# arclab-hku/ESVIO

Hardware: AMD Instinct MI355X
Metric: Mevents/s through time-surface+detect+track @640x480 (higher is better)
Workload: dtype f64 timestamps / u8 images / f32 LK sums in the reference build's order

## Files before the change

### esvio_amd/csrc/fe_api.cpp

```cpp
#include "fe_internal.h"

namespace {
typedef int (*nccl_allgather_fn)(const void*, void*, size_t, int , void* ,
                                 hipStream_t);
struct NcclId {
  char internal[128];
};
typedef int (*nccl_get_id_fn)(NcclId*);
typedef int (*nccl_init_rank_fn)(void** , int, NcclId, int);
typedef int (*nccl_destroy_fn)(void*);
void* rccl_lib() {
  static void* lib = []() -> void* {
    const char* names[] = {"librccl.so.1", "librccl.so"};
    for (const char* n : names)
      if (void* l = dlopen(n, RTLD_NOW | RTLD_NOLOAD | RTLD_GLOBAL)) return l;
    for (const char* n : names)
      if (void* l = dlopen(n, RTLD_NOW | RTLD_GLOBAL)) return l;
    return dlopen("/opt/rocm/lib/librccl.so.1", RTLD_NOW | RTLD_GLOBAL);
  }();
  return lib;
}
template <class F>
F rccl_sym(const char* name) {
  void* l = rccl_lib();
// ... 116 lines not shown
  if (hipSetDevice(dev) != hipSuccess) return ESVIO_FE_ENODEVICE;

  esvio_fe_ctx* c = new esvio_fe_ctx();
  c->cfg = *cfg;
  c->dev = dev;
  c->W = cfg->width;
  c->H = cfg->height;
  c->P = (uint32_t)c->W * c->H;
  c->invalid_key = 2 * c->P;
  c->key_bits = 1;
  while ((1ull << c->key_bits) <= (unsigned long long)c->invalid_key) c->key_bits++;
  c->hw = host::disc_halfwidths(cfg->min_dist);
  c->trace = getenv("ESVIO_FE_TRACE") != nullptr;
  if (const char* v = getenv("ESVIO_FE_SLOW_CALL_MS")) c->slow_call_ms = atof(v);
  c->mask_event.reset(c->W, c->H);

  auto bail = [&](int rc) {
    esvio_fe_destroy(c);
    return rc;
  };
  {
    int n_cu = 0;
    if (hipDeviceGetAttribute(&n_cu, hipDeviceAttributeMultiprocessorCount, dev) != hipSuccess || n_cu <= 0) {
      (void)hipGetLastError();
      n_cu = 64;
    }
    const int lk_blocks = (std::max(cfg->max_cnt, 1) + kLkPointsPerBlock - 1) / kLkPointsPerBlock;
    c->n_cu = n_cu;
    c->waits_fit_spec = lk_blocks + 2 <= n_cu;
    c->waits_fit_chain = 2 * lk_blocks + 2 <= n_cu;
// ... 3425 lines not shown
    for (int i = 0; i <= kMaxDiscR; i++) sa.hw[i] = i < (int)hw.size() ? (int8_t)hw[i] : -1;
  }
  sa.disc_c = (flags & ESVIO_FE_SELECT_TABLE) ? -1 : disc_threshold(sa.hw, sa.radius);
  if (mask) {
    host::BitMask bm;
    bm.reset(c->W, c->H);
    bm.from_bytes(mask);
    std::memcpy(pin.mask, bm.bits.data(), bm.bits.size() * 4);
    HIPCHK(c, hipMemcpyAsync(c->d_mask_bits, pin.mask, bm.bits.size() * 4, hipMemcpyHostToDevice, s));
    sa.init_bits = c->d_mask_bits;
  }
  if (n_stamp) {
    std::memcpy(pin.news, stamp_xy, (size_t)n_stamp * 8);
    sa.stamp_pts = (const float2*)zpin.news;
    sa.n_stamp = n_stamp;
  }
  pin.counts[0] = pin.counts[1] = pin.counts[2] = -1;
  sa.host_counts = zpin.counts;
  if (variant == 1) sa.one_wave = 1;
  if (variant == 2) sa.gbitmap = c->d_sel_bitmap;
  const KernelId id = launch_select_args(c, sa);
  HIPCHK(c, hipMemcpyAsync(out_xy, c->d_ptsD, (size_t)M * 8, hipMemcpyDeviceToHost, s));
  HIPCHK(c, hipMemcpyAsync(out_idx, c->d_sel_idx, (size_t)M * 4, hipMemcpyDeviceToHost, s));
  HIPCHK(c, hipStreamSynchronize(s));
  for (int i = 0; i < 3; i++) counts[i] = pin.counts[i];
  if (kernel_id) *kernel_id = (int32_t)id;
  if (c->prof_on) resolve_profile(c);
  return 0;
}

int esvio_fe_track_image_space(esvio_fe_handle c, double cur_time, const uint8_t* img_left, const uint8_t* img_right, int space,
                               int pub_this_frame, esvio_fe_tracks* out) {
  if (!c || !img_left) return ESVIO_FE_EINVAL;
  if (space != ESVIO_FE_HOST && space != ESVIO_FE_DEVICE) return fail(c, ESVIO_FE_EINVAL, "track_image_space: bad memory space");
  HIPCHK(c, hipSetDevice(c->dev));
  if (!c->announced.empty() || !c->inflight.empty())
    return fail(c, ESVIO_FE_EINVAL, "event batches are announced on this handle");
  if (int rc = track_image_impl(c, cur_time, img_left, img_right, pub_this_frame != 0, space)) return rc;
  return fill_tracks(c, out);
}

int esvio_fe_track_image(esvio_fe_handle c, double cur_time, const uint8_t* img_left,
// ... 787 lines not shown
```

### esvio_amd/csrc/fe_ctx.h

```cpp
#pragma once
#include <hip/hip_runtime.h>

#include <algorithm>
#include <atomic>
#include <chrono>
#include <cmath>
#include <cstdarg>
#include <cstdio>
#include <cstdlib>
#include <cstring>
#include <dlfcn.h>
#include <map>
#include <string>
#include <utility>
#include <deque>
#include <vector>

#include "../../include/esvio_fe.h"
#include "../../include/esvio_fe_test.h"
#include "fe_aedat.h"
#include "fe_bag.h"
#include "fe_host.h"
#include "fe_kernels.h"
#include "fe_layout.h"
// ... 273 lines not shown
  DevBuf<int32_t> d_sel_idx;
  DevBuf<uint8_t> d_fast_img;
  PinBuf<uint8_t> h_img;
  DevBuf<uint8_t> d_img;
  unsigned img_stage_next = 0;
  PinBuf<uint8_t> h_pin;

  int n_id = 0;
  double cur_time = 0, prev_time = 0;
  std::vector<P2f> prev_pts, cur_pts, cur_right_pts, n_pts;
  std::vector<P2f> cur_un_pts, cur_un_right_pts, pts_velocity, right_pts_velocity;
  std::vector<int> ids, ids_right, track_cnt, track_cnt_right;
  std::vector<int> src_idx;
  IdMap cur_un_pts_map, prev_un_pts_map, cur_un_right_pts_map, prev_un_right_pts_map;
  host::BitMask mask_event;

  DevBuf<uint8_t> d_eq_tmp;
  bool select_ok = true;
  bool select_one_wave = false;
  DevBuf<uint32_t> d_sel_bitmap;
  bool trace = false;
  double trace_phase_ms[2][ESVIO_FE_LATENCY_PHASES] = {};
  double tail_ms[2][4] = {};
  uint64_t phase_count[2] = {0, 0};
  uint64_t phase_frames = 0, tr_cand = 0, tr_new = 0, tr_detect = 0, tr_surv = 0;
  uint64_t tr_fm_class[3] = {};
  double tr_fm_ms = 0;
  double tr_fm_max_ms = 0, tr_lift_ms = 0;
  uint64_t tr_chain_launch = 0, tr_chain_used = 0, tr_chain_cancel = 0, tr_spec_used = 0;
  Event ev_dbg_sel_start;
// ... 331 lines not shown
```

### esvio_amd/csrc/fe_host.cpp

```cpp
#include "fe_host.h"

#include <algorithm>
#include <cfloat>
#include <climits>
#include <cmath>
#include <cstdio>
#include <cstdlib>
#include <cstring>

#include <atomic>
#include <chrono>
#include <condition_variable>
#include <sys/resource.h>
#include <memory>
#include <mutex>
#include <thread>

#if defined(__linux__)
#include <pthread.h>
#include <sched.h>
#endif

#if defined(__HIP_DEVICE_COMPILE__) || defined(ESVIO_NO_SIMD_CLONES)
#define ESVIO_SIMD_CLONES
// ... 107 lines not shown

void BitMask::stamp_disc(int cx, int cy, int r, const std::vector<int>& hw) {
  for (int oy = -r; oy <= r; oy++) {
    const int y = cy + oy;
    if (y < 0 || y >= H) continue;
    const int h = hw[oy < 0 ? -oy : oy];
    if (h < 0) continue;
    const int x0 = std::max(cx - h, 0), x1 = std::min(cx + h, W - 1);
    if (x1 < x0) continue;
    for (int w = x0 >> 5; w <= (x1 >> 5); w++) {
      const int lo = std::max(x0 - (w << 5), 0), hi = std::min(x1 - (w << 5), 31);
      const uint32_t m = (hi == 31 ? 0xffffffffu : ((1u << (hi + 1)) - 1u)) & ~((1u << lo) - 1u);
      bits[(size_t)y * wpr + w] |= m;
    }
  }
}

void BitMask::from_bytes(const uint8_t* mask) {
  std::fill(bits.begin(), bits.end(), 0u);
  for (int y = 0; y < H; y++)
    for (int x = 0; x < W; x++)
      if (mask[(size_t)y * W + x] == 255) bits[(size_t)y * wpr + (x >> 5)] |= 1u << (x & 31);
}

namespace {

struct OcvRng {
  uint64_t s = ~0ull;
  unsigned next() {
    s = (uint64_t)(unsigned)s * 4164903690U + (unsigned)(s >> 32);
// ... 1239 lines not shown
```

### esvio_amd/csrc/fe_host.h

```cpp
#pragma once
#include <atomic>
#include <stdint.h>

#include <vector>

#include "../../include/esvio_fe.h"
#include "../../include/esvio_fe_test.h"

namespace esvio {
inline void cpu_relax() {
#if !defined(__HIP_DEVICE_COMPILE__) && (defined(__x86_64__) || defined(__i386__))
  __builtin_ia32_pause();
#endif
}
namespace host {

int cv_round(double v);
int cv_floor(float v);

void lift_projective(const esvio_fe_camera& cam, double u, double v, double out[3]);
void lift_projective_batch(const esvio_fe_camera& cam, const float* uv, int n, double* xu, double* yu);

std::vector<int> disc_halfwidths(int r);

struct BitMask {
  int W = 0, H = 0, wpr = 0;
  std::vector<uint32_t> bits;
  void reset(int w, int h);
  bool test(int x, int y) const { return (bits[(size_t)y * wpr + (x >> 5)] >> (x & 31)) & 1u; }
  void stamp_disc(int cx, int cy, int r, const std::vector<int>& hw);
  void from_bytes(const uint8_t* mask);
};

struct RansacPool;
RansacPool* ransac_pool_create(int helpers);
void ransac_pool_destroy(RansacPool* p);
void ransac_pool_wake(RansacPool* p);
void host_hypot(const double* x, const double* y, int n, double* out);
int host_nullspace(const double* A, int n, int lanes, double* f);
struct RansacStats {
  uint64_t calls, iterations, points, ns, lmeds_calls, lmeds_ns;
};
RansacStats ransac_stats(bool reset);
void ransac_tail(uint64_t out6[6], bool reset);
void ransac_pool_hold(RansacPool* p, int mask, bool on);
void ransac_pool_set_idle_work(RansacPool* p, const std::atomic<int>* pending, bool (*fn)(void*), void* arg);
int find_fundamental_mat(const float* p1, const float* p2, int n, double thr, double conf,
                         uint8_t* status, RansacPool* pool = nullptr);
// ... 4 lines not shown
```

### esvio_amd/csrc/fe_internal.h

```cpp
#pragma once
#include "fe_ctx.h"

namespace esvio {
namespace fe {

template <class T>
void reduce_vector(std::vector<T>& v, const std::vector<uint8_t>& status) {
  int j = 0;
  for (int i = 0; i < int(v.size()); i++)
    if (status[i]) v[j++] = v[i];
  v.resize(j);
}

inline uint8_t* px00(const PyrDesc& d) { return d.img[0] + (size_t)kPad * d.stride[0] + kPad; }

inline int lookback_expired(esvio_fe_ctx* c) {
  return c->pin[0].counts[3] ? fail(c, ESVIO_FE_EINTERNAL, "radix sort look-back spin expired") : 0;
}

int ensure_event_capacity(esvio_fe_ctx* c, size_t n);
int ensure_sort_capacity(esvio_fe_ctx* c, size_t n);
int ensure_part_capacity(esvio_fe_ctx* c, size_t n, bool mc);
int ensure_cand_capacity(esvio_fe_ctx* c, int set, size_t n);
int ensure_arc_capacity(esvio_fe_ctx* c, size_t n, int set);
// ... 31 lines not shown
               int flags);
void run_lk(esvio_fe_ctx* c, const LkArgs& f, const LkArgs* b, float2* back_pts, uint8_t* back_status);
enum LkPairKind { kLkTemporal, kLkStereo };
struct LkPair {
  LkArgs f, b;
  LkOut out;
};
LkPair lk_pair(const PyrDesc& P, const PyrDesc& N, const P2f* src, const int* n_ptr, int n_max, LkPairKind kind,
               const LkOut& out);
void run_lk_pair(esvio_fe_ctx* c, const LkPair& p);
int copy_level0_out(esvio_fe_ctx* c, const PyrDesc& d, uint8_t* out);
int copy_level0_in(esvio_fe_ctx* c, const PyrDesc& d, const uint8_t* in, int space = ESVIO_FE_HOST);
bool in_border_event(const esvio_fe_ctx* c, const P2f& pt);
double pt_distance(const P2f& a, const P2f& b);
void event_set_mask(esvio_fe_ctx* c);
std::vector<P2f> undistorted_pts(const std::vector<P2f>& pts, const esvio_fe_camera& cam);
std::vector<P2f> pts_velocity_fn(std::vector<int>& ids, std::vector<P2f>& pts, IdMap& cur_id_pts,
                                 IdMap& prev_id_pts, double dt, size_t n_left);
void reject_with_f_event(esvio_fe_ctx* c);
void clear_tracker_state(esvio_fe_ctx* c);
SelectArgs make_select_args(esvio_fe_ctx* c, int set, int max_corners, float2* out_pts, int out_base,
                            int32_t* out_idx);
size_t select_lds_bytes(const esvio_fe_ctx* c);
KernelId launch_select_args(esvio_fe_ctx* c, SelectArgs s);
void compact_set(esvio_fe_ctx* c, const esvio_fe_ctx::CandSet& cs, uint32_t nblk, bool booked);
void run_select(esvio_fe_ctx* c, int set, int max_corners, float2* out_pts, int out_base, int32_t* out_idx,
                const uint32_t* mask_bits = nullptr, int* host_counts = nullptr, bool publish = false,
                const float2* stamp_pts = nullptr, int n_stamp = 0);
void run_arc(esvio_fe_ctx* c, const EventRec* ev, uint32_t n, const PyrDesc* ts, bool use_mask,
             bool want_flags, bool want_cand, int set, bool marked = false);
int run_detect(esvio_fe_ctx* c, const EventRec* ev, uint32_t n, const PyrDesc& ts, int set, bool marked);
inline size_t detect_cand_need(const esvio_fe_ctx* c, size_t n) { return c->detector == ESVIO_FE_DETECT_FAST ? (size_t)c->P : n; }
hipError_t sync_main(esvio_fe_ctx* c);
hipError_t sync_event(hipEvent_t ev);

int stager_threads_from_env();
inline bool stager_enabled(const esvio_fe_ctx* c) { return c->stage_threads > 0; }
int stager_begin(esvio_fe_ctx* c, const esvio_fe_event* left, size_t nL, const esvio_fe_event* right, size_t nR,
                 int dma_groups, int* slot_out, bool by_camera = false);
int stager_attach_left(esvio_fe_ctx* c, int slot, hipStream_t s, const EventRec** dL);
int stager_mark_read_aux(esvio_fe_ctx* c, int slot, hipStream_t s);
bool stager_ready(esvio_fe_ctx* c, int slot);
int stager_attach(esvio_fe_ctx* c, int slot, size_t nL, hipStream_t s, const EventRec** dL, const EventRec** dR);
// ... 45 lines not shown
```

### esvio_amd/csrc/fe_kernels.h

```cpp
#pragma once
#include <hip/hip_runtime.h>
#include <stdint.h>
#include <stdlib.h>

#include <vector>

namespace esvio {


struct __attribute__((aligned(16))) EventRec {
  uint16_t x, y;
  uint32_t sec, nsec;
  uint8_t pol;
  uint8_t pad[3];
};
static_assert(sizeof(EventRec) == 16, "event record must be 16 B");

constexpr int kPad = 24;
constexpr int kMaxLevels = 4;
constexpr int kLkWin = 21;
constexpr int kArcBlock = 256;
constexpr int kMaxDiscR = 63;

struct PyrDesc {
// ... 572 lines not shown
  uint32_t n;
  uint32_t tiles;
  const double* bounds;
  uint32_t n_bounds;
  uint32_t* tmax;
  SliceResult* res;
  uint32_t* cuts;
};
struct SliceArgs {
  SliceCam cam[2];
};
void launch_slice_reduce(hipStream_t s, const SliceArgs& a);
void launch_slice_scan(hipStream_t s, const SliceArgs& a);
void launch_slice_cuts(hipStream_t s, const SliceArgs& a);

struct SelectArgs {
  const uint32_t* comp_xy;
  const uint32_t* comp_idx;
  const uint32_t* total;
  int W, H, wpr;
  int max_corners;
  int radius;
  int8_t hw[kMaxDiscR + 1];
  int disc_c;
  float2* out_pts;
  int32_t* out_idx;
  int out_base;
  int* n_out;
  int* n_total;
  int* host_counts;
  uint32_t* gbitmap;
  const uint32_t* init_bits;
  const float2* stamp_pts;
  int n_stamp;
  unsigned long long* pub_slots;
  unsigned long long* pub_done;
  uint32_t pub_seq;
  int one_wave;
};
KernelId launch_select(hipStream_t s, const SelectArgs& a, size_t lds_bytes);
inline int disc_threshold(const int8_t* hw, int radius) {
  long inside = -1, outside = (long)(radius + 1) * (radius + 1);
  for (int dy = 0; dy <= radius && dy <= kMaxDiscR; dy++) {
    const long h = hw[dy];
    if (h >= 0) inside = inside > h * h + (long)dy * dy ? inside : h * h + (long)dy * dy;
    const long o = (h + 1) * (h + 1) + (long)dy * dy;
    outside = outside < o ? outside : o;
  }
  return inside >= 0 && inside < outside ? (int)inside : -1;
}

constexpr int kKfBlurTileW = 64, kKfBlurTileH = 16;
constexpr int kKfPatternTests = 256;
constexpr uint32_t kKfMatchMaxTrain = 1u << 20;
// ... 81 lines not shown
```

### esvio_amd/csrc/fe_kernels.hip

```cpp
#include "fe_kernels.h"
#include "fe_mc.h"

#include <algorithm>
#include <cstdio>
#include <cstdlib>
#include <cstring>
#include <tuple>
#include <type_traits>

namespace esvio {

namespace {
template <typename... P, typename... A>
void launch_k(void (*kernel)(P...), dim3 grid, dim3 block, unsigned shmem, hipStream_t s, A... args) {
  static_assert(sizeof...(P) == sizeof...(A), "argument count");
  hipLaunchKernelGGL(kernel, grid, block, shmem, s, args...);
}
}

__device__ __forceinline__ int lane_id() { return threadIdx.x & 63; }

__device__ __forceinline__ double ev_time(uint32_t sec, uint32_t nsec) {
  return __dadd_rn((double)sec, __dmul_rn(1e-9, (double)nsec));
}
// ... 4801 lines not shown
}

__global__ __launch_bounds__(64) void k_select(SelectArgs a) {
  extern __shared__ __attribute__((aligned(16))) uint32_t lds[];
  select_body<false>(a, lds);
}
__global__ __launch_bounds__(64) void k_select_gbm(SelectArgs a) {
  extern __shared__ __attribute__((aligned(16))) uint32_t lds[];
  select_body<true>(a, lds);
}


constexpr int kSelMwThreads = 1024;
constexpr int kSelMwQueue = kSelMwThreads + 64;
size_t select_mw_extra_lds_bytes() { return (size_t)(2 * kSelMwQueue + 32 + 16 + 128 + 64) * 4; }

__global__ __launch_bounds__(kSelMwThreads) void k_select_mw(SelectArgs a) {
  extern __shared__ __attribute__((aligned(16))) uint32_t lds[];
  const int tid = threadIdx.x, lane = tid & 63, wave = tid >> 6;
  const int nwords = a.H * a.wpr;
  uint32_t* const bitmap = lds;
  int* const hwtab = (int*)(lds + ((nwords + 3) & ~3));
  uint32_t* const spts = (uint32_t*)(hwtab + 64);
  uint32_t* const q_xy = spts + ((a.n_stamp + 3) & ~3);
  uint32_t* const q_ci = q_xy + kSelMwQueue;
  uint32_t* const wcnt = q_ci + kSelMwQueue;
  uint32_t* const ctrl = wcnt + 16;
  uint32_t* const adj = ctrl + 16;
  uint32_t* const acc_xy = adj + 128;
  const int r = a.radius;
  if (a.init_bits) {
    for (int i = tid * 4; i < nwords; i += kSelMwThreads * 4) {
      if (i + 3 < nwords) {
        *(uint4*)(bitmap + i) = *(const uint4*)(a.init_bits + i);
      } else {
        for (int k = i; k < nwords; k++) bitmap[k] = a.init_bits[k];
      }
    }
  } else {
    for (int i = tid * 4; i < nwords; i += kSelMwThreads * 4) {
      if (i + 3 < nwords) {
        *(uint4*)(bitmap + i) = make_uint4(0, 0, 0, 0);
      } else {
        for (int k = i; k < nwords; k++) bitmap[k] = 0;
      }
    }
  }
  if (tid < 64) hwtab[tid] = tid <= r ? (int)a.hw[tid] : -1;
  if (tid == 0) ctrl[0] = 0;
  if (a.stamp_pts)
    for (int k = tid; k < a.n_stamp; k += kSelMwThreads) {
      const float2 p = a.stamp_pts[k];
      spts[k] = (uint32_t)__float2int_rn(p.x) | ((uint32_t)__float2int_rn(p.y) << 16);
    }
  __syncthreads();
  if (a.stamp_pts) {
    const int rows = 2 * r + 1;
    for (int t = tid; t < a.n_stamp * rows; t += kSelMwThreads) {
      const int p = t / rows, row = t - p * rows;
      const uint32_t v = spts[p];
      const int x = (int)(v & 0xffffu), y = (int)(v >> 16);
      const int hwr = hwtab[row < r ? r - row : row - r];
      if (r <= 15) {
        stamp_row_small<false>(bitmap, a.wpr, a.W, a.H, x, y - r + row, hwr);
      } else {
        stamp_row<false>(bitmap, a.wpr, a.W, a.H, x, y - r + row, hwr);
        if (r > 31) stamp_row_tail<false>(bitmap, a.wpr, a.W, a.H, x, y - r + row, hwr);
      }
    }
  }
  const uint32_t total = *a.total;
  __syncthreads();
  uint32_t pos = 0;
  int qoff = 0, qn = 0;
  int accepted = 0;
  const uint32_t last = total ? total - 1 : 0;
  while (accepted < a.max_corners && (qn > 0 || pos < total)) {
    for (;;) {
      const bool from_q = tid < qn;
      const uint32_t si = pos + (uint32_t)(tid - qn);
      const bool have = from_q || si < total;
      uint32_t xy, ci;
      if (from_q) {
        xy = q_xy[qoff + tid];
        ci = q_ci[qoff + tid];
      } else {
        xy = a.comp_xy[min(si, last)];
        ci = a.comp_idx[min(si, last)];
      }
      const int x = xy & 0xffff, y = xy >> 16;
      const bool alive = have && !((bitmap[y * a.wpr + (x >> 5)] >> (x & 31)) & 1u);
      const lanemask_t m = bal(alive);
      if (lane == 0) wcnt[wave] = (uint32_t)__builtin_popcountll(m);
      lds_barrier();
      uint32_t before = 0, all = 0;
#pragma unroll
      for (int w = 0; w < kSelMwThreads / 64; w++) {
        const uint32_t cw = wcnt[w];
        before += w < wave ? cw : 0u;
        all += cw;
// ... 90 lines not shown
                         __ATOMIC_RELAXED, __HIP_MEMORY_SCOPE_AGENT);
    if (a.host_counts) {
      a.host_counts[0] = accepted;
      a.host_counts[1] = a.out_base + accepted;
      a.host_counts[2] = (int)total;
    }
  }
}

KernelId launch_select(hipStream_t s, const SelectArgs& a, size_t lds_bytes) {
  if (a.gbitmap) {
    launch_k(k_select_gbm, dim3(1), dim3(64), lds_bytes, s, a);
    return K_SELECT_GBM;
  }
  if (!a.one_wave && lds_bytes + select_mw_extra_lds_bytes() <= 160 * 1024) {
    launch_k(k_select_mw, dim3(1), dim3(kSelMwThreads), lds_bytes + select_mw_extra_lds_bytes(), s, a);
    return K_SELECT_MW;
  }
  launch_k(k_select, dim3(1), dim3(64), lds_bytes, s, a);
  return K_SELECT;
}

__device__ __forceinline__ uint32_t image_gray(uint32_t r, uint32_t g, uint32_t b) {
  return (r * 9798u + g * 19235u + b * 3735u + (1u << 14)) >> 15;
}
__device__ __forceinline__ uint32_t image_gray3(uint32_t v, uint32_t cls) {
  const uint32_t b0 = v & 0xffu, b1 = (v >> 8) & 0xffu, b2 = (v >> 16) & 0xffu;
  return cls == 2u ? image_gray(b2, b1, b0) : image_gray(b0, b1, b2);
}
__device__ __forceinline__ uint32_t image_gray4(uint32_t q0, uint32_t q1, uint32_t q2, uint32_t cls) {
  return image_gray3(q0, cls) | image_gray3(q0 >> 24 | q1 << 8, cls) << 8 | image_gray3(q1 >> 16 | q2 << 16, cls) << 16 |
// ... 911 lines not shown
```

### esvio_amd/csrc/fe_stages.cpp

```cpp
#include "fe_internal.h"

#include <optional>

namespace esvio {
namespace fe {


int ensure_event_capacity(esvio_fe_ctx* c, size_t n) { return c->d_ev.grow(c, n); }

static int grow_sort_buffers(esvio_fe_ctx* c, size_t cap) {
  c->sort_cap = 0;
  for (int i = 0; i < 2; i++) {
    c->keys[i].release();
    c->vals[i].release();
  }
  for (int i = 0; i < 2; i++) {
    if (int rc = c->keys[i].alloc(c, cap)) return rc;
    if (int rc = c->vals[i].alloc(c, cap)) return rc;
  }
  if (int rc = c->sae_marks.alloc(c, cap)) return rc;
  c->sort_cap = cap;
  return 0;
}

// ... 481 lines not shown
}


bool in_border_event(const esvio_fe_ctx* c, const P2f& pt) {
  const int BORDER_SIZE = 1;
  const int img_x = host::cv_round(pt.x), img_y = host::cv_round(pt.y);
  return BORDER_SIZE <= img_x && img_x < c->W - BORDER_SIZE && BORDER_SIZE <= img_y &&
         img_y < c->H - BORDER_SIZE;
}

double pt_distance(const P2f& a, const P2f& b) {
  const double dx = a.x - b.x, dy = a.y - b.y;
  return std::sqrt(dx * dx + dy * dy);
}

void event_set_mask(esvio_fe_ctx* c) {
  c->mask_event.reset(c->W, c->H);
  struct Item {
    int first;
    std::pair<P2f, int> second;
    int src;
  };
  std::vector<Item> cnt_pts_id;
  cnt_pts_id.reserve(c->cur_pts.size());
  for (unsigned int i = 0; i < c->cur_pts.size(); i++)
    cnt_pts_id.push_back(Item{c->track_cnt[i], std::make_pair(c->cur_pts[i], c->ids[i]), c->src_idx[i]});
  std::sort(cnt_pts_id.begin(), cnt_pts_id.end(),
            [](const Item& a, const Item& b) { return a.first > b.first; });
  c->cur_pts.clear();
  c->ids.clear();
  c->track_cnt.clear();
  c->src_idx.clear();
  for (auto& it : cnt_pts_id) {
    const int px = host::cv_round(it.second.first.x), py = host::cv_round(it.second.first.y);
    if (px < 0 || px >= c->W || py < 0 || py >= c->H) continue;
    if (!c->mask_event.test(px, py)) {
      c->cur_pts.push_back(it.second.first);
      c->ids.push_back(it.second.second);
      c->track_cnt.push_back(it.first);
      c->src_idx.push_back(it.src);
      c->mask_event.stamp_disc(px, py, c->cfg.min_dist, c->hw);
    }
  }
}

std::vector<P2f> undistorted_pts(const std::vector<P2f>& pts, const esvio_fe_camera& cam) {
  const size_t n = pts.size();
  std::vector<P2f> un(n);
  if (!n) return un;
  std::vector<double> lx(n), ly(n);
  host::lift_projective_batch(cam, &pts[0].x, (int)n, lx.data(), ly.data());
  for (size_t i = 0; i < n; i++) un[i] = P2f{(float)lx[i], (float)ly[i]};
  return un;
}

std::vector<P2f> pts_velocity_fn(std::vector<int>& ids, std::vector<P2f>& pts, IdMap& cur_id_pts,
                                 IdMap& prev_id_pts, double dt, size_t n_left) {
  std::vector<P2f> vel;
// ... 10 lines not shown
        vel.push_back(P2f{0, 0});
      }
    }
  } else {
    vel.assign(n_left, P2f{0, 0});
  }
  return vel;
}

void reject_with_f_event(esvio_fe_ctx* c) {
  if (c->trace) c->tr_fm_class[c->cur_pts.size() < 8 ? 0 : c->cur_pts.size() < 15 ? 1 : 2]++;
  if (c->cur_pts.size() >= 8) {
    const esvio_fe_camera& cam = c->cfg.cam[0];
    const double FOCAL = c->cfg.focal_length;
    const size_t n = c->prev_pts.size();
    std::vector<float> un_cur(n * 2), un_prev(n * 2);
    std::vector<double> lx(n), ly(n);
    const double cx = c->W / 2.0, cy = c->H / 2.0;
    const auto tl = std::chrono::steady_clock::now();
    const bool pre = c->pre_lift_valid && c->pre_lx.size() == n;
    if (!pre) host::lift_projective_batch(cam, &c->prev_pts[0].x, (int)n, lx.data(), ly.data());
    const double* plx = pre ? c->pre_lx.data() : lx.data();
    const double* ply = pre ? c->pre_ly.data() : ly.data();
    c->pre_lift_valid = false;
    for (size_t i = 0; i < n; i++) {
      un_prev[2 * i] = (float)(FOCAL * plx[i] / 1.0 + cx);
      un_prev[2 * i + 1] = (float)(FOCAL * ply[i] / 1.0 + cy);
    }
    host::lift_projective_batch(cam, &c->cur_pts[0].x, (int)n, lx.data(), ly.data());
    for (size_t i = 0; i < n; i++) {
      un_cur[2 * i] = (float)(FOCAL * lx[i] / 1.0 + cx);
      un_cur[2 * i + 1] = (float)(FOCAL * ly[i] / 1.0 + cy);
    }
    std::vector<uint8_t> status(c->cur_pts.size());
    const auto t0 = std::chrono::steady_clock::now();
    host::find_fundamental_mat(un_prev.data(), un_cur.data(), (int)c->cur_pts.size(),
                               c->cfg.f_threshold, 0.99, status.data(), c->pool);
    if (c->trace) {
      const double ms = std::chrono::duration<double, std::milli>(std::chrono::steady_clock::now() - t0).count();
      c->tr_fm_ms += ms;
      c->tr_fm_max_ms = std::max(c->tr_fm_max_ms, ms);
      c->tr_lift_ms += std::chrono::duration<double, std::milli>(t0 - tl).count();
    }
    reduce_vector(c->prev_pts, status);
    reduce_vector(c->cur_pts, status);
    reduce_vector(c->ids, status);
    reduce_vector(c->track_cnt, status);
    reduce_vector(c->src_idx, status);
  }
// ... 40 lines not shown
  s.out_pts = out_pts;
  s.out_idx = out_idx;
  s.out_base = out_base;
  s.n_out = c->dres.counts;
  s.n_total = c->dres.counts + 1;
  s.host_counts = nullptr;
  s.init_bits = nullptr;
  s.gbitmap = nullptr;
  s.pub_slots = nullptr;
  s.pub_done = nullptr;
  s.pub_seq = 0;
  s.one_wave = c->select_one_wave ? 1 : 0;
  return s;
}

size_t select_lds_bytes(const esvio_fe_ctx* c) {
  return ((size_t)c->H * ((c->W + 31) / 32) + 4 + 64 + (size_t)std::max(c->cfg.max_cnt, 1)) * 4;
}
static size_t select_tables_lds_bytes(const esvio_fe_ctx* c) {
  return (4 + 64 + (size_t)std::max(c->cfg.max_cnt, 1)) * 4;
}

KernelId launch_select_args(esvio_fe_ctx* c, SelectArgs s) {
  if (!c->select_ok) s.gbitmap = c->d_sel_bitmap;
  ScopedKernel k(c, K_SELECT_MW, 0);
  const KernelId id = launch_select(cur_stream(c), s, s.gbitmap ? select_tables_lds_bytes(c) : select_lds_bytes(c));
  k.id = id;
  return id;
}

void compact_set(esvio_fe_ctx* c, const esvio_fe_ctx::CandSet& cs, uint32_t nblk, bool booked) {
  std::optional<ScopedKernel> k;
  if (booked) k.emplace(c, K_COMPACT, 0);
  launch_compact(cur_stream(c), cs.xy, cs.idx, cs.cnt, nblk, cs.comp_xy, cs.comp_idx, cs.total, booked ? cs.grp.p : nullptr);
}

void run_select(esvio_fe_ctx* c, int set, int max_corners, float2* out_pts, int out_base,
                int32_t* out_idx, const uint32_t* mask_bits, int* host_counts, bool publish,
                const float2* stamp_pts, int n_stamp) {
  SelectArgs s = make_select_args(c, set, max_corners, out_pts, out_base, out_idx);
  s.host_counts = host_counts;
  s.init_bits = mask_bits;
  s.stamp_pts = stamp_pts;
  s.n_stamp = n_stamp;
  if (publish) {
    s.pub_slots = c->d_pub_slots;
    s.pub_done = c->d_pub_done;
    s.pub_seq = c->pub_seq;
  }
  launch_select_args(c, s);
}

void run_arc(esvio_fe_ctx* c, const EventRec* ev, uint32_t n, const PyrDesc* ts, bool use_mask,
             bool want_flags, bool want_cand, int set, bool marked) {
  ArcArgs a{};
  a.ev = ev;
  a.n = n;
  a.L2 = c->L2;
  a.S2 = c->S2;
// ... 67 lines not shown
```

### esvio_amd/csrc/fe_track.cpp

```cpp
#include "fe_internal.h"

#include <sched.h>
#include <sys/resource.h>

#include <atomic>
#include <condition_variable>
#include <mutex>
#include <thread>

namespace esvio {
namespace fe {

struct PrefetchJob {
  Inflight b;
  bool wait_planes = false;
  int lks_wait = -1;
};

static int prefetch_issue(esvio_fe_ctx* c, const PrefetchJob& j) {
  const Inflight& b = j.b;
  StreamScope on_prefetch_stream(c->stream2);
  PrefetchBatchScope its_event_images(&b);
  if (j.wait_planes) HIPCHK(c, hipStreamWaitEvent(c->stream2, c->ev_planes_free, 0));
  if (j.lks_wait >= 0) HIPCHK(c, hipStreamWaitEvent(c->stream2, c->ev_lks_done[j.lks_wait], 0));
// ... 856 lines not shown
      const int n_max_cnt = M - n_kept;
      if (int rc = upload_kept()) return rc;
      if (n_max_cnt <= 0 && will_spec && n_kept)
        if (const Inflight* nb = next_batch())
          if (int rc = enqueue_spec_temporal(c, *nb, n_kept, false)) return rc;
      if (n_max_cnt > 0) {
        detect = true;
        if (!will_spec && n_kept) std::memcpy(pin.news, c->cur_pts.data(), (size_t)n_kept * 8);
        if (arc_prefetched) HIPCHK(c, hipStreamWaitEvent(c->stream, c->ev_lane_arc[arc_lane], 0));
        c->pub_seq++;
        if (c->trace) {
          HIPCHK(c, hipEventRecord(c->ev_dbg_sel_start, cur_stream(c)));
          c->tr_sel_launch = clk::now();
        }
        run_select(c, c->cand_cur, n_max_cnt, (float2*)zpin.news, n_kept, nullptr, nullptr, zpin.counts, will_spec,
                   (const float2*)zpin.news, n_kept);
        sub(PH_PUB_SELECT);
        if (will_spec)
          if (const Inflight* nb = next_batch())
            if (int rc = enqueue_spec_temporal(c, *nb, n_kept, true)) return rc;
        sub(PH_PUB_SPEC);
        HIPCHK(c, hipEventRecord(c->ev_sel_host, cur_stream(c)));
        if (int rc = finalize_pending(c)) return rc;
        if (!c->pend_right.active || c->pend_right.left.empty() ||
            (!c->lazy_late && event_over(c->ev_lks_done[c->pend_right.set])))
          if (int rc = finalize_right(c)) return rc;
        sub(PH_PUB_PREV_RIGHT);
        if (split_right) HIPCHK(c, hipStreamWaitEvent(c->stream, c->ev_right_ready, 0));
        run_lk_pair(c, lk_pair(curL, curR, zpin.news + n_kept, c->dres.counts, n_max_cnt, kLkStereo, zpin.s2));
        if (c->lazy_new) HIPCHK(c, hipEventRecord(c->ev_lknew_done, cur_stream(c)));
        sub(PH_PUB_STEREO_NEW);
// ... 219 lines not shown
```

### esvio_amd/frontend.py

```python
import ctypes as C
import os

import numpy as np

from . import build as _build

_HERE = os.path.dirname(os.path.abspath(__file__))
HOST, DEVICE = 0, 1
EVENT_IMAGES_AHEAD = 2
LK_USE_INITIAL_FLOW = 4


class FrontendError(RuntimeError):
    pass


class Camera(C.Structure):
    _fields_ = [(n, C.c_double) for n in ("fx", "fy", "cx", "cy", "k1", "k2", "p1", "p2")]


class Config(C.Structure):
    _fields_ = [
        ("width", C.c_int32), ("height", C.c_int32),
        ("decay_ms", C.c_double),
# ... 284 lines not shown
    "esvio_fe_kf_describe",
    "esvio_fe_bow_vocabulary_header", "esvio_fe_bow_set_vocabulary", "esvio_fe_bow_transform", "esvio_fe_bow_add",
    "esvio_fe_bow_query", "esvio_fe_bow_detect_loop", "esvio_fe_bow_clear", "esvio_fe_bow_entries", "esvio_fe_bow_reserve",
    "esvio_fe_bow_create_vocabulary", "esvio_fe_bow_get_created",
]
TEST_SYMBOLS = [
    "esvio_fe_build_pyramid", "esvio_fe_debug_counters", "esvio_fe_debug_inject", "esvio_fe_device_memory",
    "esvio_fe_export_level",
    "esvio_fe_find_fundamental_mat_held", "esvio_fe_find_fundamental_mat_idle", "esvio_fe_find_fundamental_mat_mt",
    "esvio_fe_get_kernel_stats", "esvio_fe_host_hypot", "esvio_fe_host_nullspace", "esvio_fe_host_stage_copy",
    "esvio_fe_host_stage_pack", "esvio_fe_staging_counters",
    "esvio_fe_kernel_count", "esvio_fe_kernel_name", "esvio_fe_latency_phase_name", "esvio_fe_latency_recent",
    "esvio_fe_latency_stats", "esvio_fe_lift_projective", "esvio_fe_plain_call_counters", "esvio_fe_ransac_stats",
    "esvio_fe_ransac_tail", "esvio_fe_raw_tile_bytes", "esvio_fe_reset_kernel_stats", "esvio_fe_select_candidates",
    "esvio_fe_set_profiling", "esvio_fe_set_sae",
    "esvio_fe_slice_tile_events", "esvio_fe_stage_kernel_count", "esvio_fe_stream",
    "esvio_fe_aedat_tile_events", "esvio_fe_ingest_kernel_count", "esvio_fe_aedat_walk_tap", "esvio_fe_aedat_walk_state_bytes",
    "esvio_fe_bag_tile_events", "esvio_fe_bag_walk_tap", "esvio_fe_bag_walk_state_bytes",
    "esvio_fe_bag_image_walk_tap", "esvio_fe_image_tile_pixels", "esvio_fe_event_image_kernel_stats",
    "esvio_fe_aedat_frame_walk_tap", "esvio_fe_aedat_frame_kernel_stats", "esvio_fe_frame16_tile_pixels",
    "esvio_fe_kf_kernel_count", "esvio_fe_kf_kernel_name", "esvio_fe_kf_kernel_stats", "esvio_fe_kf_blur_tile",
    "esvio_fe_bow_kernel_count", "esvio_fe_bow_kernel_name", "esvio_fe_bow_kernel_stats", "esvio_fe_bow_limits", "esvio_fe_bow_scores",
    "esvio_fe_bow_create_kernel_count", "esvio_fe_bow_create_kernel_name", "esvio_fe_bow_create_kernel_stats", "esvio_fe_bow_create_pick",
]

LATENCY_PHASES = 16
SELECT_EUCLID, SELECT_TABLE = 1, 2


class LatencyCall(C.Structure):
# ... 143 lines not shown
    L.esvio_fe_mem_alloc.argtypes = [i, sz, vp]
    L.esvio_fe_mem_free.argtypes = [i, vp]
    L.esvio_fe_mem_upload.argtypes = [vp, vp, sz]
    L.esvio_fe_register_host_buffer.argtypes = [vp, sz]
    L.esvio_fe_unregister_host_buffer.argtypes = [vp]
    L.esvio_fe_debug_inject.argtypes = [vp, i]
    L.esvio_fe_debug_counters.argtypes = [vp, vp]
    L.esvio_fe_plain_call_counters.argtypes = [vp, vp]
    L.esvio_fe_good_features_to_track.argtypes = [vp, vp, i, d, d, vp, vp, vp, vp]
    L.esvio_fe_track_image.argtypes = [vp, d, vp, vp, i, vp]
    L.esvio_fe_pack_track_records.argtypes = [vp, vp, vp]
    L.esvio_fe_set_lazy_new_stereo.argtypes = [vp, i]
    L.esvio_fe_set_host_threads.argtypes = [vp, i]
    L.esvio_fe_ransac_stats.argtypes = [vp, i]
    L.esvio_fe_host_hypot.argtypes = [vp, vp, i, vp]
    L.esvio_fe_host_stage_copy.argtypes = [vp, vp, C.c_size_t]
    L.esvio_fe_host_nullspace.argtypes = [vp, i, i, vp, C.POINTER(C.c_int32)]
    L.esvio_fe_find_fundamental_mat_mt.argtypes = [vp, vp, i, d, d, i, vp, C.POINTER(C.c_int32)]
    L.esvio_fe_finish.argtypes = [vp, vp]
    L.esvio_fe_get_time_surface.argtypes = [vp, i, vp]
    L.esvio_fe_export_image.argtypes = [vp, i, vp, i]
    L.esvio_fe_import_image.argtypes = [vp, i, vp, i]
    L.esvio_fe_export_level.argtypes = [vp, i, i, vp, vp, C.POINTER(C.c_int32), C.POINTER(C.c_int32), C.POINTER(C.c_int32)]
    L.esvio_fe_fast_corners.argtypes = [vp, i, vp, i, i, i, i, vp, vp, C.c_int32, C.POINTER(C.c_int32),
                                        C.POINTER(C.c_int32)]
    L.esvio_fe_set_detector.argtypes = [vp, i, i]
    L.esvio_fe_set_event_images.argtypes = [vp, i]
    L.esvio_fe_clear_event_images.argtypes = [vp]
    L.esvio_fe_get_event_image.argtypes = [vp, i, vp, i]
    L.esvio_fe_get_event_canvas.argtypes = [vp, vp, i]
# ... 1560 lines not shown
    if rc != 0:
        raise FrontendError("host_nullspace rc=%d" % rc)
    return f, redone.value


def host_hypot(x, y):
    x = np.ascontiguousarray(x, np.float64)
    y = np.ascontiguousarray(y, np.float64)
    out = np.empty_like(x)
    rc = load_library().esvio_fe_host_hypot(_p(x), _p(y), x.size, _p(out))
    if rc != 0:
        raise FrontendError("host_hypot rc=%d" % rc)
    return out


def ransac_stats(reset=False):
    out = (C.c_uint64 * 6)()
    L = load_library()
    rc = L.esvio_fe_ransac_stats(out, 1 if reset else 0)
    if rc != 0:
        raise FrontendError("ransac_stats rc=%d" % rc)
    return {"calls": int(out[0]), "iterations": int(out[1]), "points": int(out[2]), "us": out[3] / 1e3,
            "lmeds_calls": int(out[4]), "lmeds_us": out[5] / 1e3}


def ransac_tail(reset=False):
    out = (C.c_uint64 * 6)()
    rc = load_library().esvio_fe_ransac_tail(out, 1 if reset else 0)
    if rc != 0:
        raise FrontendError("ransac_tail rc=%d" % rc)
# ... 159 lines not shown
```

Before: 3014.

## Use spatial grid for host set_mask, stage select candidates in LDS, pass stamps in args

The host-side non-max set_mask switches from stamping discs into a full-frame bitmask to a sparse cell grid that checks neighbouring cells, so the per-frame bitmap clear and disc stamping go away. The select kernel prefetches up to a fixed number of candidates into LDS at kernel start, and kept-point pixel coordinates are packed into the kernel arguments instead of being read from pinned host memory. Fundamental-matrix scratch vectors are also reused across frames instead of reallocated. A test tap compares the grid and bitmap forms. The risks are a larger argument struct, extra LDS use that may lower occupancy, and possible divergence between the grid and bitmap semantics.

```diff
diff --git a/esvio_amd/csrc/fe_api.cpp b/esvio_amd/csrc/fe_api.cpp
--- a/esvio_amd/csrc/fe_api.cpp
+++ b/esvio_amd/csrc/fe_api.cpp
@@ -154,6 +154,7 @@
   c->trace = getenv("ESVIO_FE_TRACE") != nullptr;
   if (const char* v = getenv("ESVIO_FE_SLOW_CALL_MS")) c->slow_call_ms = atof(v);
   c->mask_event.reset(c->W, c->H);
+  c->mask_grid.size(c->W, c->H, cfg->min_dist);
 
   auto bail = [&](int rc) {
     esvio_fe_destroy(c);
@@ -3609,7 +3610,12 @@
     std::memcpy(pin.news, stamp_xy, (size_t)n_stamp * 8);
     sa.stamp_pts = (const float2*)zpin.news;
     sa.n_stamp = n_stamp;
-  }
+    std::vector<uint32_t> px((size_t)n_stamp);
+    for (int i = 0; i < n_stamp; i++)
+      px[i] = (uint32_t)host::cv_round(stamp_xy[2 * i]) | ((uint32_t)host::cv_round(stamp_xy[2 * i + 1]) << 16);
+    set_select_stamp_px(sa, px.data());
+  }
+  sa.stage_n = (int)std::min<size_t>(cs.cap, (size_t)kSelStage);
   pin.counts[0] = pin.counts[1] = pin.counts[2] = -1;
   sa.host_counts = zpin.counts;
   if (variant == 1) sa.one_wave = 1;
@@ -3621,6 +3627,44 @@
   for (int i = 0; i < 3; i++) counts[i] = pin.counts[i];
   if (kernel_id) *kernel_id = (int32_t)id;
   if (c->prof_on) resolve_profile(c);
+  return 0;
+}
+
+struct esvio_fe_set_mask_tap {
+  int W, H, r;
+  std::vector<int> hw;
+  host::DiscGrid grid;
+  host::BitMask bm;
+};
+void* esvio_fe_set_mask_tap_create(int width, int height, int min_dist) {
+  if (width < 1 || height < 1 || width > 65535 || height > 65535 || min_dist < 1 || min_dist > kMaxDiscR) return nullptr;
+  auto* t = new esvio_fe_set_mask_tap{width, height, min_dist, host::disc_halfwidths(min_dist), {}, {}};
+  return t;
+}
+void esvio_fe_set_mask_tap_destroy(void* tap) { delete (esvio_fe_set_mask_tap*)tap; }
+int esvio_fe_set_mask_tap_run(void* tap, const float* pts, const int32_t* track_cnt, const int32_t* ids, int n,
+                              int32_t* keep_bitmap, int32_t* keep_grid, uint32_t* px_grid, int32_t counts[2]) {
+  auto* t = (esvio_fe_set_mask_tap*)tap;
+  if (!t || n < 0 || !counts || (n && (!pts || !track_cnt || !ids || !keep_bitmap || !keep_grid || !px_grid)))
+    return ESVIO_FE_EINVAL;
+  for (int form = 0; form < 2; form++) {
+    std::vector<P2f> p((size_t)n);
+    std::vector<int> id(ids, ids + n), cnt(track_cnt, track_cnt + n), src((size_t)n);
+    for (int i = 0; i < n; i++) {
+      p[i] = P2f{pts[2 * i], pts[2 * i + 1]};
+      src[i] = i;
+    }
+    set_mask_lists(t->W, t->H, t->r, t->hw, p, id, cnt, src, form ? &t->grid : nullptr, form ? nullptr : &t->bm);
+    for (size_t k = 0; k < src.size(); k++)
+      if (std::memcmp(&p[k], pts + 2 * src[k], 8) != 0 || id[k] != ids[src[k]] || cnt[k] != track_cnt[src[k]])
+        return ESVIO_FE_EINTERNAL;
+    std::copy(src.begin(), src.end(), form ? keep_grid : keep_bitmap);
+    counts[form] = (int32_t)src.size();
+    if (form) {
+      if (t->grid.px.size() != src.size()) return ESVIO_FE_EINTERNAL;
+      std::copy(t->grid.px.begin(), t->grid.px.end(), px_grid);
+    }
+  }
   return 0;
 }
 
diff --git a/esvio_amd/csrc/fe_ctx.h b/esvio_amd/csrc/fe_ctx.h
--- a/esvio_amd/csrc/fe_ctx.h
+++ b/esvio_amd/csrc/fe_ctx.h
@@ -311,6 +311,10 @@
   std::vector<int> src_idx;
   IdMap cur_un_pts_map, prev_un_pts_map, cur_un_right_pts_map, prev_un_right_pts_map;
   host::BitMask mask_event;
+  host::DiscGrid mask_grid;
+  std::vector<float> fm_un_cur, fm_un_prev;
+  std::vector<double> fm_lx, fm_ly;
+  std::vector<uint8_t> fm_status;
 
   DevBuf<uint8_t> d_eq_tmp;
   bool select_ok = true;
diff --git a/esvio_amd/csrc/fe_host.cpp b/esvio_amd/csrc/fe_host.cpp
--- a/esvio_amd/csrc/fe_host.cpp
+++ b/esvio_amd/csrc/fe_host.cpp
@@ -145,6 +145,46 @@
       bits[(size_t)y * wpr + w] |= m;
     }
   }
+}
+
+void DiscGrid::size(int w, int h, int radius) {
+  if (w == W && h == H && radius == r) return;
+  W = w;
+  H = h;
+  r = radius;
+  side = std::max(radius, 0) + 1;
+  gw = (w + side - 1) / side;
+  gh = (h + side - 1) / side;
+  head.assign((size_t)gw * gh, -1);
+  next.clear();
+  touched.clear();
+  px.clear();
+}
+
+void DiscGrid::clear() {
+  for (const int32_t cell : touched) head[cell] = -1;
+  touched.clear();
+  next.clear();
+  px.clear();
+}
+
+bool DiscGrid::blocked(int x, int y, const std::vector<int>& hw) const {
+  const int cx = x / side, cy = y / side;
+  for (int gy = std::max(cy - 1, 0); gy <= std::min(cy + 1, gh - 1); gy++)
+    for (int gx = std::max(cx - 1, 0); gx <= std::min(cx + 1, gw - 1); gx++)
+      for (int32_t k = head[(size_t)gy * gw + gx]; k >= 0; k = next[k]) {
+        const int dx = std::abs(x - (int)(px[k] & 0xffffu)), dy = std::abs(y - (int)(px[k] >> 16));
+        if (dy <= r && dx <= hw[dy]) return true;
+      }
+  return false;
+}
+
+void DiscGrid::add(int x, int y) {
+  const int32_t cell = (y / side) * gw + x / side;
+  if (head[cell] < 0) touched.push_back(cell);
+  next.push_back(head[cell]);
+  head[cell] = (int32_t)px.size();
+  px.push_back((uint32_t)x | ((uint32_t)y << 16));
 }
 
 void BitMask::from_bytes(const uint8_t* mask) {
diff --git a/esvio_amd/csrc/fe_host.h b/esvio_amd/csrc/fe_host.h
--- a/esvio_amd/csrc/fe_host.h
+++ b/esvio_amd/csrc/fe_host.h
@@ -32,6 +32,18 @@
   void from_bytes(const uint8_t* mask);
 };
 
+struct DiscGrid {
+  int W = 0, H = 0, r = -1, side = 1, gw = 0, gh = 0;
+  std::vector<int32_t> head;
+  std::vector<int32_t> next;
+  std::vector<int32_t> touched;
+  std::vector<uint32_t> px;
+  void size(int w, int h, int radius);
+  void clear();
+  bool blocked(int x, int y, const std::vector<int>& hw) const;
+  void add(int x, int y);
+};
+
 struct RansacPool;
 RansacPool* ransac_pool_create(int helpers);
 void ransac_pool_destroy(RansacPool* p);
diff --git a/esvio_amd/csrc/fe_internal.h b/esvio_amd/csrc/fe_internal.h
--- a/esvio_amd/csrc/fe_internal.h
+++ b/esvio_amd/csrc/fe_internal.h
@@ -69,6 +69,8 @@
 bool in_border_event(const esvio_fe_ctx* c, const P2f& pt);
 double pt_distance(const P2f& a, const P2f& b);
 void event_set_mask(esvio_fe_ctx* c);
+void set_mask_lists(int W, int H, int r, const std::vector<int>& hw, std::vector<P2f>& pts, std::vector<int>& ids,
+                    std::vector<int>& track_cnt, std::vector<int>& src_idx, host::DiscGrid* grid, host::BitMask* bm);
 std::vector<P2f> undistorted_pts(const std::vector<P2f>& pts, const esvio_fe_camera& cam);
 std::vector<P2f> pts_velocity_fn(std::vector<int>& ids, std::vector<P2f>& pts, IdMap& cur_id_pts,
                                  IdMap& prev_id_pts, double dt, size_t n_left);
@@ -81,7 +83,8 @@
 void compact_set(esvio_fe_ctx* c, const esvio_fe_ctx::CandSet& cs, uint32_t nblk, bool booked);
 void run_select(esvio_fe_ctx* c, int set, int max_corners, float2* out_pts, int out_base, int32_t* out_idx,
                 const uint32_t* mask_bits = nullptr, int* host_counts = nullptr, bool publish = false,
-                const float2* stamp_pts = nullptr, int n_stamp = 0);
+                const float2* stamp_pts = nullptr, int n_stamp = 0, const uint32_t* stamp_px = nullptr);
+void set_select_stamp_px(SelectArgs& s, const uint32_t* stamp_px);
 void run_arc(esvio_fe_ctx* c, const EventRec* ev, uint32_t n, const PyrDesc* ts, bool use_mask,
              bool want_flags, bool want_cand, int set, bool marked = false);
 int run_detect(esvio_fe_ctx* c, const EventRec* ev, uint32_t n, const PyrDesc& ts, int set, bool marked);
diff --git a/esvio_amd/csrc/fe_kernels.h b/esvio_amd/csrc/fe_kernels.h
--- a/esvio_amd/csrc/fe_kernels.h
+++ b/esvio_amd/csrc/fe_kernels.h
@@ -610,6 +610,8 @@
 void launch_slice_scan(hipStream_t s, const SliceArgs& a);
 void launch_slice_cuts(hipStream_t s, const SliceArgs& a);
 
+constexpr int kSelArgPts = 256;
+constexpr int kSelStage = 4096;
 struct SelectArgs {
   const uint32_t* comp_xy;
   const uint32_t* comp_idx;
@@ -629,11 +631,15 @@
   const uint32_t* init_bits;
   const float2* stamp_pts;
   int n_stamp;
+  int stamp_in_args;
+  int stage_n;
+  uint32_t stamp_px[kSelArgPts];
   unsigned long long* pub_slots;
   unsigned long long* pub_done;
   uint32_t pub_seq;
   int one_wave;
 };
+static_assert(sizeof(SelectArgs) <= 1536, "SelectArgs travels by value: well under the 4 KB of kernel arguments");
 KernelId launch_select(hipStream_t s, const SelectArgs& a, size_t lds_bytes);
 inline int disc_threshold(const int8_t* hw, int radius) {
   long inside = -1, outside = (long)(radius + 1) * (radius + 1);
diff --git a/esvio_amd/csrc/fe_kernels.hip b/esvio_amd/csrc/fe_kernels.hip
--- a/esvio_amd/csrc/fe_kernels.hip
+++ b/esvio_amd/csrc/fe_kernels.hip
@@ -4839,6 +4839,7 @@
 constexpr int kSelMwThreads = 1024;
 constexpr int kSelMwQueue = kSelMwThreads + 64;
 size_t select_mw_extra_lds_bytes() { return (size_t)(2 * kSelMwQueue + 32 + 16 + 128 + 64) * 4; }
+static_assert(kSelStage % kSelMwThreads == 0 && kSelArgPts <= kSelMwThreads, "a thread stages kSelStage / threads candidates, one kept point");
 
 __global__ __launch_bounds__(kSelMwThreads) void k_select_mw(SelectArgs a) {
   extern __shared__ __attribute__((aligned(16))) uint32_t lds[];
@@ -4853,7 +4854,24 @@
   uint32_t* const ctrl = wcnt + 16;
   uint32_t* const adj = ctrl + 16;
   uint32_t* const acc_xy = adj + 128;
+  uint32_t* const st_xy = acc_xy + 64;
+  uint32_t* const st_ci = st_xy + a.stage_n;
   const int r = a.radius;
+  const uint32_t stage_n = (uint32_t)a.stage_n;
+  constexpr int kStagePer = kSelStage / kSelMwThreads;
+  uint32_t pf_xy[kStagePer], pf_ci[kStagePer];
+  if (stage_n) {
+#pragma unroll
+    for (int k = 0; k < kStagePer; k++) {
+      const uint32_t i = min((uint32_t)(tid + k * kSelMwThreads), stage_n - 1);
+      pf_xy[k] = a.comp_xy[i];
+      pf_ci[k] = a.comp_idx[i];
+    }
+  }
+  const uint32_t total = *a.total;
+  const bool stamps = a.n_stamp > 0 && (a.stamp_in_args || a.stamp_pts);
+  uint32_t pf_stamp = 0;
+  if (a.stamp_in_args && tid < a.n_stamp) pf_stamp = a.stamp_px[tid];
   if (a.init_bits) {
     for (int i = tid * 4; i < nwords; i += kSelMwThreads * 4) {
       if (i + 3 < nwords) {
@@ -4873,13 +4891,26 @@
   }
   if (tid < 64) hwtab[tid] = tid <= r ? (int)a.hw[tid] : -1;
   if (tid == 0) ctrl[0] = 0;
-  if (a.stamp_pts)
+  if (stage_n) {
+#pragma unroll
+    for (int k = 0; k < kStagePer; k++) {
+      const uint32_t i = (uint32_t)(tid + k * kSelMwThreads);
+      if (i < stage_n) {
+        st_xy[i] = pf_xy[k];
+        st_ci[i] = pf_ci[k];
+      }
+    }
+  }
+  if (a.stamp_in_args) {
+    if (tid < a.n_stamp) spts[tid] = pf_stamp;
+  } else if (stamps) {
     for (int k = tid; k < a.n_stamp; k += kSelMwThreads) {
       const float2 p = a.stamp_pts[k];
       spts[k] = (uint32_t)__float2int_rn(p.x) | ((uint32_t)__float2int_rn(p.y) << 16);
     }
-  __syncthreads();
-  if (a.stamp_pts) {
+  }
+  __syncthreads();
+  if (stamps) {
     const int rows = 2 * r + 1;
     for (int t = tid; t < a.n_stamp * rows; t += kSelMwThreads) {
       const int p = t / rows, row = t - p * rows;
@@ -4894,7 +4925,6 @@
       }
     }
   }
-  const uint32_t total = *a.total;
   __syncthreads();
   uint32_t pos = 0;
   int qoff = 0, qn = 0;
@@ -4909,6 +4939,9 @@
       if (from_q) {
         xy = q_xy[qoff + tid];
         ci = q_ci[qoff + tid];
+      } else if (si < stage_n) {
+        xy = have ? st_xy[si] : 0u;
+        ci = st_ci[si];
       } else {
         xy = a.comp_xy[min(si, last)];
         ci = a.comp_idx[min(si, last)];
@@ -5029,7 +5062,11 @@
     return K_SELECT_GBM;
   }
   if (!a.one_wave && lds_bytes + select_mw_extra_lds_bytes() <= 160 * 1024) {
-    launch_k(k_select_mw, dim3(1), dim3(kSelMwThreads), lds_bytes + select_mw_extra_lds_bytes(), s, a);
+    SelectArgs m = a;
+    const size_t base = lds_bytes + select_mw_extra_lds_bytes();
+    const size_t room = (160 * 1024 - base) / 8 / kSelMwThreads * kSelMwThreads;
+    m.stage_n = (int)std::min<size_t>((size_t)std::min(std::max(a.stage_n, 0), kSelStage), room);
+    launch_k(k_select_mw, dim3(1), dim3(kSelMwThreads), base + (size_t)m.stage_n * 8, s, m);
     return K_SELECT_MW;
   }
   launch_k(k_select, dim3(1), dim3(64), lds_bytes, s, a);
diff --git a/esvio_amd/csrc/fe_stages.cpp b/esvio_amd/csrc/fe_stages.cpp
--- a/esvio_amd/csrc/fe_stages.cpp
+++ b/esvio_amd/csrc/fe_stages.cpp
@@ -519,34 +519,47 @@
   return std::sqrt(dx * dx + dy * dy);
 }
 
-void event_set_mask(esvio_fe_ctx* c) {
-  c->mask_event.reset(c->W, c->H);
+void set_mask_lists(int W, int H, int r, const std::vector<int>& hw, std::vector<P2f>& pts, std::vector<int>& ids,
+                    std::vector<int>& track_cnt, std::vector<int>& src_idx, host::DiscGrid* grid, host::BitMask* bm) {
+  if (grid) {
+    grid->size(W, H, r);
+    grid->clear();
+  } else {
+    bm->reset(W, H);
+  }
   struct Item {
     int first;
     std::pair<P2f, int> second;
     int src;
   };
   std::vector<Item> cnt_pts_id;
-  cnt_pts_id.reserve(c->cur_pts.size());
-  for (unsigned int i = 0; i < c->cur_pts.size(); i++)
-    cnt_pts_id.push_back(Item{c->track_cnt[i], std::make_pair(c->cur_pts[i], c->ids[i]), c->src_idx[i]});
+  cnt_pts_id.reserve(pts.size());
+  for (unsigned int i = 0; i < pts.size(); i++)
+    cnt_pts_id.push_back(Item{track_cnt[i], std::make_pair(pts[i], ids[i]), src_idx[i]});
   std::sort(cnt_pts_id.begin(), cnt_pts_id.end(),
             [](const Item& a, const Item& b) { return a.first > b.first; });
-  c->cur_pts.clear();
-  c->ids.clear();
-  c->track_cnt.clear();
-  c->src_idx.clear();
+  pts.clear();
+  ids.clear();
+  track_cnt.clear();
+  src_idx.clear();
   for (auto& it : cnt_pts_id) {
     const int px = host::cv_round(it.second.first.x), py = host::cv_round(it.second.first.y);
-    if (px < 0 || px >= c->W || py < 0 || py >= c->H) continue;
-    if (!c->mask_event.test(px, py)) {
-      c->cur_pts.push_back(it.second.first);
-      c->ids.push_back(it.second.second);
-      c->track_cnt.push_back(it.first);
-      c->src_idx.push_back(it.src);
-      c->mask_event.stamp_disc(px, py, c->cfg.min_dist, c->hw);
+    if (px < 0 || px >= W || py < 0 || py >= H) continue;
+    if (!(grid ? grid->blocked(px, py, hw) : bm->test(px, py))) {
+      pts.push_back(it.second.first);
+      ids.push_back(it.second.second);
+      track_cnt.push_back(it.first);
+      src_idx.push_back(it.src);
+      if (grid)
+        grid->add(px, py);
+      else
+        bm->stamp_disc(px, py, r, hw);
     }
   }
+}
+
+void event_set_mask(esvio_fe_ctx* c) {
+  set_mask_lists(c->W, c->H, c->cfg.min_dist, c->hw, c->cur_pts, c->ids, c->track_cnt, c->src_idx, &c->mask_grid, nullptr);
 }
 
 std::vector<P2f> undistorted_pts(const std::vector<P2f>& pts, const esvio_fe_camera& cam) {
@@ -587,8 +600,14 @@
     const esvio_fe_camera& cam = c->cfg.cam[0];
     const double FOCAL = c->cfg.focal_length;
     const size_t n = c->prev_pts.size();
-    std::vector<float> un_cur(n * 2), un_prev(n * 2);
-    std::vector<double> lx(n), ly(n);
+    std::vector<float>&un_cur = c->fm_un_cur, &un_prev = c->fm_un_prev;
+    std::vector<double>&lx = c->fm_lx, &ly = c->fm_ly;
+    std::vector<uint8_t>& status = c->fm_status;
+    un_cur.resize(n * 2);
+    un_prev.resize(n * 2);
+    lx.resize(n);
+    ly.resize(n);
+    status.resize(c->cur_pts.size());
     const double cx = c->W / 2.0, cy = c->H / 2.0;
     const auto tl = std::chrono::steady_clock::now();
     const bool pre = c->pre_lift_valid && c->pre_lx.size() == n;
@@ -605,7 +624,6 @@
       un_cur[2 * i] = (float)(FOCAL * lx[i] / 1.0 + cx);
       un_cur[2 * i + 1] = (float)(FOCAL * ly[i] / 1.0 + cy);
     }
-    std::vector<uint8_t> status(c->cur_pts.size());
     const auto t0 = std::chrono::steady_clock::now();
     host::find_fundamental_mat(un_prev.data(), un_cur.data(), (int)c->cur_pts.size(),
                                c->cfg.f_threshold, 0.99, status.data(), c->pool);
@@ -676,6 +694,11 @@
   return s;
 }
 
+void set_select_stamp_px(SelectArgs& s, const uint32_t* stamp_px) {
+  s.stamp_in_args = stamp_px && s.n_stamp > 0 && s.n_stamp <= kSelArgPts;
+  if (s.stamp_in_args) std::memcpy(s.stamp_px, stamp_px, (size_t)s.n_stamp * 4);
+}
+
 size_t select_lds_bytes(const esvio_fe_ctx* c) {
   return ((size_t)c->H * ((c->W + 31) / 32) + 4 + 64 + (size_t)std::max(c->cfg.max_cnt, 1)) * 4;
 }
@@ -699,12 +722,14 @@
 
 void run_select(esvio_fe_ctx* c, int set, int max_corners, float2* out_pts, int out_base,
                 int32_t* out_idx, const uint32_t* mask_bits, int* host_counts, bool publish,
-                const float2* stamp_pts, int n_stamp) {
+                const float2* stamp_pts, int n_stamp, const uint32_t* stamp_px) {
   SelectArgs s = make_select_args(c, set, max_corners, out_pts, out_base, out_idx);
   s.host_counts = host_counts;
   s.init_bits = mask_bits;
   s.stamp_pts = stamp_pts;
   s.n_stamp = n_stamp;
+  set_select_stamp_px(s, stamp_px);
+  s.stage_n = (int)std::min<size_t>(c->cand[set].cap, (size_t)kSelStage);
   if (publish) {
     s.pub_slots = c->d_pub_slots;
     s.pub_done = c->d_pub_done;
diff --git a/esvio_amd/csrc/fe_track.cpp b/esvio_amd/csrc/fe_track.cpp
--- a/esvio_amd/csrc/fe_track.cpp
+++ b/esvio_amd/csrc/fe_track.cpp
@@ -894,7 +894,7 @@
           c->tr_sel_launch = clk::now();
         }
         run_select(c, c->cand_cur, n_max_cnt, (float2*)zpin.news, n_kept, nullptr, nullptr, zpin.counts, will_spec,
-                   (const float2*)zpin.news, n_kept);
+                   (const float2*)zpin.news, n_kept, c->mask_grid.px.data());
         sub(PH_PUB_SELECT);
         if (will_spec)
           if (const Inflight* nb = next_batch())
diff --git a/esvio_amd/frontend.py b/esvio_amd/frontend.py
--- a/esvio_amd/frontend.py
+++ b/esvio_amd/frontend.py
@@ -322,6 +322,7 @@
     "esvio_fe_latency_stats", "esvio_fe_lift_projective", "esvio_fe_plain_call_counters", "esvio_fe_ransac_stats",
     "esvio_fe_ransac_tail", "esvio_fe_raw_tile_bytes", "esvio_fe_reset_kernel_stats", "esvio_fe_select_candidates",
     "esvio_fe_set_profiling", "esvio_fe_set_sae",
+    "esvio_fe_set_mask_tap_create", "esvio_fe_set_mask_tap_destroy", "esvio_fe_set_mask_tap_run",
     "esvio_fe_slice_tile_events", "esvio_fe_stage_kernel_count", "esvio_fe_stream",
     "esvio_fe_aedat_tile_events", "esvio_fe_ingest_kernel_count", "esvio_fe_aedat_walk_tap", "esvio_fe_aedat_walk_state_bytes",
     "esvio_fe_bag_tile_events", "esvio_fe_bag_walk_tap", "esvio_fe_bag_walk_state_bytes",
@@ -495,6 +496,11 @@
     L.esvio_fe_set_host_threads.argtypes = [vp, i]
     L.esvio_fe_ransac_stats.argtypes = [vp, i]
     L.esvio_fe_host_hypot.argtypes = [vp, vp, i, vp]
+    L.esvio_fe_set_mask_tap_create.argtypes = [i, i, i]
+    L.esvio_fe_set_mask_tap_create.restype = vp
+    L.esvio_fe_set_mask_tap_destroy.argtypes = [vp]
+    L.esvio_fe_set_mask_tap_destroy.restype = None
+    L.esvio_fe_set_mask_tap_run.argtypes = [vp, vp, vp, vp, i, vp, vp, vp, vp]
     L.esvio_fe_host_stage_copy.argtypes = [vp, vp, C.c_size_t]
     L.esvio_fe_host_nullspace.argtypes = [vp, i, i, vp, C.POINTER(C.c_int32)]
     L.esvio_fe_find_fundamental_mat_mt.argtypes = [vp, vp, i, d, d, i, vp, C.POINTER(C.c_int32)]
@@ -2085,6 +2091,33 @@
     return out
 
 
+class SetMaskTap:
+
+    def __init__(self, width, height, min_dist):
+        self.L = load_library()
+        self.h = self.L.esvio_fe_set_mask_tap_create(int(width), int(height), int(min_dist))
+        if not self.h:
+            raise FrontendError("set_mask_tap_create(%d, %d, %d)" % (width, height, min_dist))
+
+    def run(self, pts, track_cnt, ids):
+        pts = np.ascontiguousarray(pts, np.float32).reshape(-1, 2)
+        cnt = np.ascontiguousarray(track_cnt, np.int32).reshape(-1)
+        ids = np.ascontiguousarray(ids, np.int32).reshape(-1)
+        n = pts.shape[0]
+        assert cnt.size == n and ids.size == n
+        kb, kg, px = np.full(n, -1, np.int32), np.full(n, -1, np.int32), np.zeros(n, np.uint32)
+        counts = np.zeros(2, np.int32)
+        rc = self.L.esvio_fe_set_mask_tap_run(self.h, _p(pts), _p(cnt), _p(ids), n, _p(kb), _p(kg), _p(px), _p(counts))
+        if rc != 0:
+            raise FrontendError("set_mask_tap_run rc=%d" % rc)
+        return kb[:counts[0]].copy(), kg[:counts[1]].copy(), px[:counts[1]].copy()
+
+    def close(self):
+        if self.h:
+            self.L.esvio_fe_set_mask_tap_destroy(self.h)
+            self.h = None
+
+
 def ransac_stats(reset=False):
     out = (C.c_uint64 * 6)()
     L = load_library()
```

Measured after the change: 2883. 4.3% lower.
